# facebookresearch/dpr-scale

Measured on NVIDIA H100. Metric: query+ctx pairs/sec (BERT-base, seq128), higher is better.
Workload: dtype bf16

## Files before the change

dpr_scale_b200/csrc/common.cuh:

```cuda
#pragma once
#include <cuda.h>
#include <cuda_runtime.h>
#include <cuda_bf16.h>
#include <cuda_fp16.h>
#include <stdint.h>
#include "wgmma.cuh"

#ifndef DPRB_HANG_GUARD
#define DPRB_HANG_GUARD 1
#endif

namespace dprb {

typedef __nv_bfloat16 bf16;

void set_last_error(const char* fmt, ...);
#define DPRB_CHECK_CUDA(expr)                                                        \
  do {                                                                               \
    cudaError_t _e = (expr);                                                         \
    if (_e != cudaSuccess) {                                                         \
      dprb::set_last_error("%s:%d CUDA error %d (%s) in `%s`", __FILE__, __LINE__,   \
                           (int)_e, cudaGetErrorString(_e), #expr);                  \
      return 2;                                                                      \
    }                                                                                \
  } while (0)
#define DPRB_REQUIRE(cond, ...)                                                      \
  do {                                                                               \
    if (!(cond)) {                                                                   \
      dprb::set_last_error(__VA_ARGS__);                                             \
      return 1;                                                                      \
    }                                                                                \
  } while (0)

int num_sms();
#define DPRB_NUM_SMS(var)           \
  const int var = dprb::num_sms();  \
  if (var <= 0) return 2

void count_launch();
#define DPRB_LAUNCH_CHECK()                \
  do {                                     \
    dprb::count_launch();                  \
    DPRB_CHECK_CUDA(cudaGetLastError());   \
  } while (0)

__device__ __forceinline__ uint32_t smem_u32(const void* p) {
  return static_cast<uint32_t>(__cvta_generic_to_shared(p));
}
__device__ __forceinline__ uint8_t* align1024(uint8_t* p) {
  return reinterpret_cast<uint8_t*>((reinterpret_cast<uintptr_t>(p) + 1023) & ~uintptr_t(1023));
}
__device__ __forceinline__ void named_bar_sync(int id, int n) { asm volatile("bar.sync %0, %1;" ::"r"(id), "r"(n) : "memory"); }

__device__ __forceinline__ float warp_sum(float v) {
#pragma unroll
  for (int o = 16; o > 0; o >>= 1) v += __shfl_xor_sync(0xffffffffu, v, o);
  return v;
}
__device__ __forceinline__ float warp_max(float v) {
#pragma unroll
  for (int o = 16; o > 0; o >>= 1) v = fmaxf(v, __shfl_xor_sync(0xffffffffu, v, o));
  return v;
}

__device__ __forceinline__ uint32_t pack_bf16x2(float lo, float hi) {
  __nv_bfloat162 t = __floats2bfloat162_rn(lo, hi);
  return *reinterpret_cast<uint32_t*>(&t);
}
__device__ __forceinline__ float2 unpack_bf16x2(uint32_t u) {
  __nv_bfloat162 t = *reinterpret_cast<__nv_bfloat162*>(&u);
  return __bfloat1622float2(t);
}

__device__ __forceinline__ uint32_t pack_f16x2(float lo, float hi) {
  __half2 t = __floats2half2_rn(lo, hi);
  return *reinterpret_cast<uint32_t*>(&t);
}
__device__ __forceinline__ float2 unpack_f16x2(uint32_t u) {
  __half2 t = *reinterpret_cast<__half2*>(&u);
  return __half22float2(t);
}
__device__ __forceinline__ uint32_t pack_16x2(float lo, float hi, bool f16) { return f16 ? pack_f16x2(lo, hi) : pack_bf16x2(lo, hi); }
__device__ __forceinline__ float2 unpack_16x2(uint32_t u, bool f16) { return f16 ? unpack_f16x2(u) : unpack_bf16x2(u); }

__device__ __forceinline__ float2 ffma2(float2 a, float2 b, float2 c) {
  return make_float2(__fmaf_rn(a.x, b.x, c.x), __fmaf_rn(a.y, b.y, c.y));
}
__device__ __forceinline__ float2 fmul2(float2 a, float2 b) { return make_float2(__fmul_rn(a.x, b.x), __fmul_rn(a.y, b.y)); }
__device__ __forceinline__ float2 fadd2(float2 a, float2 b) { return make_float2(__fadd_rn(a.x, b.x), __fadd_rn(a.y, b.y)); }

__device__ __forceinline__ float ex2_approx(float x) {
  float y;
  asm("ex2.approx.ftz.f32 %0, %1;" : "=f"(y) : "f"(x));
  return y;
}
__device__ __forceinline__ float lg2_approx(float x) {
  float y;
  asm("lg2.approx.ftz.f32 %0, %1;" : "=f"(y) : "f"(x));
  return y;
}
__device__ __forceinline__ float rcp_approx(float x) {
  float y;
  asm("rcp.approx.ftz.f32 %0, %1;" : "=f"(y) : "f"(x));
  return y;
}
__device__ __forceinline__ void gelu_and_grad(float x, float& g, float& gd) {
  const float xc = fminf(fmaxf(x, -8.f), 8.f);
  const float x2 = xc * xc;
  float pz = fmaf(x2, 1.03455483e-3f, -1.06900513e-1f);
  pz = fmaf(pz, x2, -2.30098511f);
  const float e = ex2_approx(pz * xc);
  const float sg = rcp_approx(1.f + e);
  float zp = fmaf(x2, -3.58549371e-3f, 2.22293380e-1f);
  zp = fmaf(zp, x2, 1.59492135f);
  const float inside = (x == xc) ? zp : 0.f;
  g = x * sg;
  gd = sg * fmaf(xc * e * sg, inside, 1.f);
}
__device__ __forceinline__ void gelu_and_grad2(float2 x, float2& g, float2& gd) {
  float2 x2 = fmul2(x, x);
  x2.x = fminf(x2.x, 64.f);
  x2.y = fminf(x2.y, 64.f);
  const float2 one = make_float2(1.f, 1.f);
  float2 pz = ffma2(x2, make_float2(1.03455483e-3f, 1.03455483e-3f), make_float2(-1.06900513e-1f, -1.06900513e-1f));
  pz = ffma2(pz, x2, make_float2(-2.30098511f, -2.30098511f));
  const float2 ex = fmul2(pz, x);
  const float2 e = make_float2(ex2_approx(ex.x), ex2_approx(ex.y));
  const float2 den = fadd2(e, one);
  const float2 sg = make_float2(rcp_approx(den.x), rcp_approx(den.y));
  float2 zp = ffma2(x2, make_float2(-3.58549371e-3f, -3.58549371e-3f), make_float2(2.22293380e-1f, 2.22293380e-1f));
  zp = ffma2(zp, x2, make_float2(1.59492135f, 1.59492135f));
  g = fmul2(x, sg);
  const float2 t = ffma2(sg, make_float2(-1.f, -1.f), one);
  const float2 w = ffma2(fmul2(x, t), zp, one);
  gd = fmul2(sg, w);
}
struct Drop {
  uint32_t seed;
  uint32_t thresh16;
  float scale;
  uint32_t row_mul;
  __host__ __device__ bool on() const { return thresh16 != 0u; }
  __device__ __forceinline__ uint32_t group_mix(uint32_t r, uint32_t c8) const {
    uint32_t x = (r * row_mul) * 0x9E3779B1u + c8 * 0x85EBCA6Bu + seed;
    x ^= x >> 16; x *= 0x7FEB352Du; x ^= x >> 15;
    return x;
  }
  __device__ __forceinline__ static uint32_t pair_word(uint32_t x, uint32_t w) {
    const uint32_t k = w == 0u ? 0x846CA68Bu : (w == 1u ? 0xC2B2AE35u : (w == 2u ? 0x27D4EB2Fu : 0x165667B1u));
    uint32_t h = x * k;
    h ^= h >> 16;
    return h;
  }
  __device__ __forceinline__ uint32_t pair_hash(uint32_t r, uint32_t c_even) const {
    return pair_word(group_mix(r, c_even >> 3), (c_even >> 1) & 3u);
  }
  __device__ __forceinline__ void lanes(uint32_t h, float& m0, float& m1) const {
    m0 = (h & 0xFFFFu) >= thresh16 ? scale : 0.f;
    m1 = (h >> 16) >= thresh16 ? scale : 0.f;
  }
  __device__ __forceinline__ void mul2(uint32_t r, uint32_t c_even, float& m0, float& m1) const {
    lanes(pair_hash(r, c_even), m0, m1);
  }
  __device__ __forceinline__ void mul8(uint32_t r, uint32_t c0, float2 (&m)[4]) const {
    const uint32_t x = group_mix(r, c0 >> 3);
#pragma unroll
    for (int w = 0; w < 4; ++w) lanes(pair_word(x, (uint32_t)w), m[w].x, m[w].y);
  }
};
__device__ __forceinline__ float drop_one(const Drop& d, uint32_t r, uint32_t c) {
  float m0, m1;
  d.mul2(r, c & ~1u, m0, m1);
  return (c & 1u) ? m1 : m0;
}
inline Drop make_drop(float p, uint64_t seed, int layer, int site) {
  const uint64_t s64 = seed + (uint64_t)(layer * 8 + site + 1) * 0x9E3779B97F4A7C15ull;
  Drop d;
  d.seed = (uint32_t)(s64 ^ (s64 >> 32));
  d.thresh16 = (p > 0.f) ? (uint32_t)((double)p * 65536.0 + 0.5) : 0u;
  if (d.thresh16 > 65535u) d.thresh16 = 65535u;
  d.scale = d.thresh16 ? 1.f / (1.f - (float)d.thresh16 / 65536.f) : 1.f;
  d.row_mul = 1u;
  return d;
}
inline uint64_t drop_site_seed64(uint64_t seed, int layer, int site) { return make_drop(0.5f, seed, layer, site).seed; }
inline Drop drop_from_site(float p, uint64_t site_seed) {
  Drop d = make_drop(p, 0, 0, 0);
  d.seed = (uint32_t)site_seed;
  d.row_mul = (uint32_t)(site_seed >> 32) ? (uint32_t)(site_seed >> 32) : 1u;
  return d;
}
enum { DROP_SITE_EMBED = 0, DROP_SITE_ATTN = 1, DROP_SITE_ATTN_OUT = 2, DROP_SITE_FFN_OUT = 3,
       DROP_SITE_HEAD = 4, DROP_SITE_HEAD_IN = 5 };

__device__ __forceinline__ void mbar_init(uint64_t* bar, uint32_t count) {
  asm volatile("mbarrier.init.shared::cta.b64 [%0], %1;" ::"r"(smem_u32(bar)), "r"(count) : "memory");
}
__device__ __forceinline__ void fence_barrier_init() {
  asm volatile("fence.mbarrier_init.release.cluster;" ::: "memory");
}
__device__ __forceinline__ void fence_proxy_async_smem() {
  asm volatile("fence.proxy.async.shared::cta;" ::: "memory");
}
__device__ __forceinline__ void mbar_arrive_expect_tx(uint64_t* bar, uint32_t tx_bytes) {
  asm volatile("mbarrier.arrive.expect_tx.shared::cta.b64 _, [%0], %1;" ::"r"(smem_u32(bar)), "r"(tx_bytes)
// ... 86 lines not shown
```

dpr_scale_b200/csrc/gemm_wgmma.cu:

```cuda
#include <cstdlib>
#include <vector>
#include "common.cuh"
#include "dprb_internal.h"

namespace dprb {

namespace {

constexpr int BLOCK_M = 128;
constexpr int BLOCK_N = 256;
constexpr int BLOCK_K = 64;
constexpr int STAGES = 3;
constexpr int A_TILE_BYTES = BLOCK_M * BLOCK_K * 2;
constexpr int B_TILE_BYTES = BLOCK_N * BLOCK_K * 2;
constexpr int STAGE_BYTES = A_TILE_BYTES + B_TILE_BYTES;
constexpr int NUM_CONSUMERS = 2;
constexpr int NUM_THREADS = (NUM_CONSUMERS + 1) * 128;
constexpr int WG_ROWS = BLOCK_M / NUM_CONSUMERS;
constexpr int SUB_COLS = 64;
constexpr int SUB_BYTES = WG_ROWS * SUB_COLS * 2;
constexpr int STG_BYTES = WG_ROWS * BLOCK_N * 2;
constexpr int SMEM_BYTES = STAGES * STAGE_BYTES + NUM_CONSUMERS * STG_BYTES + 1024  + 128 ;
static_assert(SMEM_BYTES <= 227 * 1024, "ring + staging must fit one CTA per SM");
constexpr int PRODUCER_REGS = 40, CONSUMER_REGS = 232;
static_assert(128 * PRODUCER_REGS + NUM_CONSUMERS * 128 * CONSUMER_REGS <= 65536, "register file");

struct GemmParams {
  int M, N, K;
  int num_m_blocks, num_n_blocks;
  int k_blocks_total, k_blocks_per_split, splits;
  int units;
  int epilogue;
  void* D;
  long long ldd;
  const float* bias;
  int has_aux;
  int has_out2;
  float alpha;
  float* colsum;
  Drop drop;
  int aux_f16, out_f16;
  int save_pre;
};

struct Unit {
  int m0, n0, kb0, kb1;
};
__device__ __forceinline__ Unit unit_at(const GemmParams& p, int u) {
  const int tiles = p.num_m_blocks * p.num_n_blocks;
  const int tile = u % tiles, split = u / tiles;
  Unit w;
  w.m0 = (tile / p.num_n_blocks) * BLOCK_M;
  w.n0 = (tile % p.num_n_blocks) * BLOCK_N;
  w.kb0 = split * p.k_blocks_per_split;
  w.kb1 = min(w.kb0 + p.k_blocks_per_split, p.k_blocks_total);
  return w;
}

__device__ __forceinline__ void red_add_v2_f32(float* p, float a, float b) {
  asm volatile("red.global.add.v2.f32 [%0], {%1, %2};" ::"l"(p), "f"(a), "f"(b) : "memory");
}
__device__ __forceinline__ void wg_bar(int wg) { asm volatile("bar.sync %0, 128;" ::"r"(wg + 1) : "memory"); }

template <int A_MN, int B_MN, int F16>
__device__ __forceinline__ void mma_kblock(float (&acc)[128], uint32_t sa, uint32_t sb, int accumulate_first) {
  const uint64_t da = make_wgmma_desc_sw128(sa, A_MN ? BLOCK_K * 128 : 16, 1024);
  const uint64_t db = make_wgmma_desc_sw128(sb, B_MN ? BLOCK_K * 128 : 16, 1024);
  constexpr uint32_t A_KSTEP = (A_MN ? 16 * 128 : 32) >> 4;
  constexpr uint32_t B_KSTEP = (B_MN ? 16 * 128 : 32) >> 4;
#pragma unroll
  for (int k = 0; k < BLOCK_K / 16; ++k) {
    const int accum = (k > 0 || accumulate_first) ? 1 : 0;
    if (F16) wgmma_m64n256_ss_f16<A_MN, B_MN>(acc, da + k * A_KSTEP, db + k * B_KSTEP, accum);
    else wgmma_m64n256_ss_bf16<A_MN, B_MN>(acc, da + k * A_KSTEP, db + k * B_KSTEP, accum);
  }
}

__device__ __forceinline__ uint32_t pack_out(float a, float b, bool f16) { return f16 ? pack_f16x2(a, b) : pack_bf16x2(a, b); }

__device__ __forceinline__ uint32_t slab_base(const uint8_t* stg, int lr, int q) {
  return smem_u32(stg) + lr * 128 + ((lr & 7) << 4) + 4 * q;
}
__device__ __forceinline__ uint32_t slab_pair(uint32_t base, int c, int h) {
  return (base ^ ((c & 7) << 4)) + (c >> 3) * SUB_BYTES + h * 8 * 128;
}
__device__ __forceinline__ void sts32(uint32_t a, uint32_t v) { asm volatile("st.shared.b32 [%0], %1;" ::"r"(a), "r"(v)); }
__device__ __forceinline__ uint32_t lds32(uint32_t a) {
  uint32_t v;
  asm volatile("ld.shared.b32 %0, [%1];" : "=r"(v) : "r"(a));
  return v;
}
__device__ __forceinline__ int slab_boxes(int row0, int n0, int M, int N) {
  return row0 < M ? min(BLOCK_N / SUB_COLS, (N - n0 + SUB_COLS - 1) / SUB_COLS) : 0;
}
__device__ __forceinline__ void slab_tma_store(const CUtensorMap* m, const uint8_t* stg, int row0, int n0, int M, int N) {
  const int boxes = slab_boxes(row0, n0, M, N);
  for (int s = 0; s < boxes; ++s) tma_store_2d(m, smem_u32(stg + s * SUB_BYTES), n0 + s * SUB_COLS, row0);
  tma_store_commit();
}

template <bool ATOMIC>
__device__ __forceinline__ void epilogue_f32(const GemmParams& p, const float (&acc)[128], int row0, int n0, int lr, int q) {
#pragma unroll
  for (int h = 0; h < 2; ++h) {
    const int row = row0 + lr + 8 * h;
    if (row >= p.M) continue;
    float* drow = reinterpret_cast<float*>(p.D) + (long long)row * p.ldd;
#pragma unroll
    for (int c = 0; c < 32; ++c) {
      const int col = n0 + 8 * c + 2 * q;
      const float x = acc[4 * c + 2 * h] * p.alpha, y = acc[4 * c + 2 * h + 1] * p.alpha;
      if (ATOMIC) {
        if (col + 1 < p.N) red_add_v2_f32(drow + col, x, y);
        else if (col < p.N) atomicAdd(drow + col, x);
      } else {
        if (col < p.N) drow[col] = x + (p.bias != nullptr ? __ldg(p.bias + col) : 0.f);
        if (col + 1 < p.N) drow[col + 1] = y + (p.bias != nullptr ? __ldg(p.bias + col + 1) : 0.f);
      }
    }
  }
}

template <int EP, bool DROP, bool COLSUM>
__device__ __forceinline__ void epilogue16(const GemmParams& p, float (&acc)[128], uint32_t slab, int row0, int n0, int lr,
                                           int q, int lane) {
  const bool out_f16 = p.out_f16 != 0, aux_f16 = p.aux_f16 != 0;
#pragma unroll
  for (int c = 0; c < 32; ++c) {
    const int col = n0 + 8 * c + 2 * q;
    float2 b = make_float2(0.f, 0.f);
    if (p.bias != nullptr) {
      if (col + 1 < p.N) b = __ldg(reinterpret_cast<const float2*>(p.bias + col));
      else if (col < p.N) b.x = __ldg(p.bias + col);
    }
    float cs0 = 0.f, cs1 = 0.f;
#pragma unroll
    for (int h = 0; h < 2; ++h) {
      const int row = row0 + lr + 8 * h;
      const uint32_t sp = slab_pair(slab, c, h);
      float2 v = ffma2(make_float2(acc[4 * c + 2 * h], acc[4 * c + 2 * h + 1]), make_float2(p.alpha, p.alpha), b);
      if constexpr (EP == DPRB_EPI_BIAS_GELU) {
        float2 g, d;
        gelu_and_grad2(v, g, d);
        if (p.save_pre) d = v;
        sts32(sp, pack_bf16x2(g.x, g.y));
        acc[4 * c + 2 * h] = d.x;
        acc[4 * c + 2 * h + 1] = d.y;
        continue;
      }
      if constexpr (DROP) {
        float m0f, m1f;
        p.drop.mul2((uint32_t)row, (uint32_t)col, m0f, m1f);
        v.x *= m0f; v.y *= m1f;
      }
      if constexpr (EP == DPRB_EPI_BIAS_RESIDUAL) {
        const float2 a = unpack_16x2(lds32(sp), aux_f16);
        v.x += a.x; v.y += a.y;
      } else if constexpr (EP == DPRB_EPI_DGELU) {
        const float2 a = unpack_bf16x2(lds32(sp));
        v.x *= a.x; v.y *= a.y;
      } else if constexpr (EP == DPRB_EPI_DGELU_PRE) {
        float2 g, d;
        gelu_and_grad2(unpack_bf16x2(lds32(sp)), g, d);
        v.x *= d.x; v.y *= d.y;
      }
      const uint32_t o = pack_out(v.x, v.y, out_f16);
      sts32(sp, o);
      if (COLSUM && row < p.M && col < p.N) {
        const float2 f = unpack_bf16x2(o);
        cs0 += f.x;
        if (col + 1 < p.N) cs1 += f.y;
      }
    }
    if (COLSUM) {
#pragma unroll
      for (int o = 4; o < 32; o <<= 1) {
        cs0 += __shfl_xor_sync(0xFFFFFFFFu, cs0, o);
        cs1 += __shfl_xor_sync(0xFFFFFFFFu, cs1, o);
      }
      if (lane < 4) {
        if (col < p.N) atomicAdd(p.colsum + col, cs0);
        if (col + 1 < p.N) atomicAdd(p.colsum + col + 1, cs1);
      }
    }
  }
}

template <int A_MN, int B_MN, int F16>
__global__ void __launch_bounds__(NUM_THREADS, 1)
gemm_bf16_kernel(const __grid_constant__ CUtensorMap tmap_a, const __grid_constant__ CUtensorMap tmap_b,
                 const __grid_constant__ CUtensorMap tmap_d, const __grid_constant__ CUtensorMap tmap_aux,
                 const __grid_constant__ CUtensorMap tmap_out2, const GemmParams p) {
  extern __shared__ uint8_t smem_raw[];
  uint8_t* smem = align1024(smem_raw);
  uint8_t* staging = smem + STAGES * STAGE_BYTES;
  uint64_t* full_bar = reinterpret_cast<uint64_t*>(staging + NUM_CONSUMERS * STG_BYTES);
  uint64_t* empty_bar = full_bar + STAGES;
  uint64_t* aux_full = empty_bar + STAGES;
  uint64_t* slab_empty = aux_full + NUM_CONSUMERS;

  const int warp = threadIdx.x >> 5;
  const int lane = threadIdx.x & 31;
  const bool out16 = p.epilogue != DPRB_EPI_F32_ATOMIC_ADD && p.epilogue != DPRB_EPI_F32_STORE;

  if (threadIdx.x == 0) {
    tma_prefetch_desc(&tmap_a);
    tma_prefetch_desc(&tmap_b);
    if (out16) tma_prefetch_desc(&tmap_d);
    if (p.has_aux) tma_prefetch_desc(&tmap_aux);
    if (p.has_out2) tma_prefetch_desc(&tmap_out2);
    for (int i = 0; i < STAGES; ++i) {
      mbar_init(&full_bar[i], 1);
      mbar_init(&empty_bar[i], NUM_CONSUMERS * 4);
    }
    for (int i = 0; i < NUM_CONSUMERS; ++i) {
      mbar_init(&aux_full[i], 1);
      mbar_init(&slab_empty[i], 1);
    }
    fence_barrier_init();
  }
  __syncthreads();

  if (warp < 4) {
    asm volatile("setmaxnreg.dec.sync.aligned.u32 %0;" ::"n"(PRODUCER_REGS));
    if (warp == 0 && lane == 0) {
      int stage = 0;
      uint32_t phase = 0, uphase = 0;
      for (int u = blockIdx.x; u < p.units; u += gridDim.x, uphase ^= 1) {
        const Unit w = unit_at(p, u);
        const int aux_kb = min(w.kb0 + 2, w.kb1 - 1);
        for (int kb = w.kb0; kb < w.kb1; ++kb) {
          mbar_wait(&empty_bar[stage], phase ^ 1);
          mbar_arrive_expect_tx(&full_bar[stage], STAGE_BYTES);
          uint8_t* sa = smem + stage * STAGE_BYTES;
          uint8_t* sb = sa + A_TILE_BYTES;
          if (A_MN == 0) {
            tma_load_2d(sa, &tmap_a, &full_bar[stage], kb * BLOCK_K, w.m0);
          } else {
#pragma unroll
            for (int i = 0; i < BLOCK_M / 64; ++i) tma_load_2d(sa + i * (BLOCK_K * 128), &tmap_a, &full_bar[stage], w.m0 + i * 64, kb * BLOCK_K);
          }
          if (B_MN == 0) {
            tma_load_2d(sb, &tmap_b, &full_bar[stage], kb * BLOCK_K, w.n0);
          } else {
#pragma unroll
            for (int i = 0; i < BLOCK_N / 64; ++i) tma_load_2d(sb + i * (BLOCK_K * 128), &tmap_b, &full_bar[stage], w.n0 + i * 64, kb * BLOCK_K);
          }
          if (++stage == STAGES) { stage = 0; phase ^= 1; }
          if (p.has_aux && kb == aux_kb) {
            for (int g = 0; g < NUM_CONSUMERS; ++g) {
              const int row0 = w.m0 + g * WG_ROWS;
              const int boxes = slab_boxes(row0, w.n0, p.M, p.N);
              uint8_t* slab = staging + g * STG_BYTES;
              mbar_wait(&slab_empty[g], uphase);
              mbar_arrive_expect_tx(&aux_full[g], boxes * SUB_BYTES);
              for (int s = 0; s < boxes; ++s)
                tma_load_2d(slab + s * SUB_BYTES, &tmap_aux, &aux_full[g], w.n0 + s * SUB_COLS, row0);
            }
          }
        }
      }
    }
    return;
  }

  asm volatile("setmaxnreg.inc.sync.aligned.u32 %0;" ::"n"(CONSUMER_REGS));
  const int wg = (warp >> 2) - 1;
  const int t = threadIdx.x - 128 * (wg + 1);
  uint8_t* stg = staging + wg * STG_BYTES;
  const uint32_t a_off = (uint32_t)wg * (A_MN ? BLOCK_K * 128 : 64 * 128);
  const int q = lane & 3;
  const int lr = (warp & 3) * 16 + (lane >> 2);
  const uint32_t slab = slab_base(stg, lr, q);
  const int ep = p.epilogue;

  float acc[128];
  int stage = 0;
  uint32_t phase = 0, uphase = 0;
  for (int u = blockIdx.x; u < p.units; u += gridDim.x, uphase ^= 1) {
    const Unit w = unit_at(p, u);
    {
      int prev = -1;
      const int release_kb = min(w.kb0 + 1, w.kb1 - 1);
      for (int kb = w.kb0; kb < w.kb1; ++kb) {
        mbar_wait(&full_bar[stage], phase);
        const uint32_t sa = smem_u32(smem + stage * STAGE_BYTES) + a_off;
        const uint32_t sb = smem_u32(smem + stage * STAGE_BYTES + A_TILE_BYTES);
        wgmma_fence();
        mma_kblock<A_MN, B_MN, F16>(acc, sa, sb, kb > w.kb0);
        wgmma_commit();
        wgmma_wait<1>();
        if (prev >= 0) {
          __syncwarp();
          if (lane == 0) mbar_arrive(&empty_bar[prev]);
        }
        if (p.has_aux && kb == release_kb && t == 0) {
          tma_store_wait_read();
          mbar_arrive(&slab_empty[wg]);
        }
        prev = stage;
        if (++stage == STAGES) { stage = 0; phase ^= 1; }
      }
      wgmma_wait<0>();
      __syncwarp();
      if (lane == 0) mbar_arrive(&empty_bar[prev]);
    }

    const int row0 = w.m0 + wg * WG_ROWS;
    switch (ep) {
      case DPRB_EPI_F32_ATOMIC_ADD: epilogue_f32<true>(p, acc, row0, w.n0, lr, q); continue;
      case DPRB_EPI_F32_STORE: epilogue_f32<false>(p, acc, row0, w.n0, lr, q); continue;
      default: break;
    }
    if (p.has_aux) mbar_wait(&aux_full[wg], uphase);
    else if (t == 0) tma_store_wait_read();
    wg_bar(wg);
    const bool cs = p.colsum != nullptr, drop = p.drop.on();
    switch (ep) {
      case DPRB_EPI_BIAS:
        if (cs) epilogue16<DPRB_EPI_BIAS, false, true>(p, acc, slab, row0, w.n0, lr, q, lane);
        else epilogue16<DPRB_EPI_BIAS, false, false>(p, acc, slab, row0, w.n0, lr, q, lane);
        break;
      case DPRB_EPI_BIAS_GELU: epilogue16<DPRB_EPI_BIAS_GELU, false, false>(p, acc, slab, row0, w.n0, lr, q, lane); break;
      case DPRB_EPI_BIAS_RESIDUAL:
        if (drop) {
          if (cs) epilogue16<DPRB_EPI_BIAS_RESIDUAL, true, true>(p, acc, slab, row0, w.n0, lr, q, lane);
          else epilogue16<DPRB_EPI_BIAS_RESIDUAL, true, false>(p, acc, slab, row0, w.n0, lr, q, lane);
        } else {
          if (cs) epilogue16<DPRB_EPI_BIAS_RESIDUAL, false, true>(p, acc, slab, row0, w.n0, lr, q, lane);
          else epilogue16<DPRB_EPI_BIAS_RESIDUAL, false, false>(p, acc, slab, row0, w.n0, lr, q, lane);
        }
        break;
      case DPRB_EPI_DGELU:
        if (cs) epilogue16<DPRB_EPI_DGELU, false, true>(p, acc, slab, row0, w.n0, lr, q, lane);
        else epilogue16<DPRB_EPI_DGELU, false, false>(p, acc, slab, row0, w.n0, lr, q, lane);
        break;
      default:
        if (cs) epilogue16<DPRB_EPI_DGELU_PRE, false, true>(p, acc, slab, row0, w.n0, lr, q, lane);
        else epilogue16<DPRB_EPI_DGELU_PRE, false, false>(p, acc, slab, row0, w.n0, lr, q, lane);
        break;
    }
    fence_proxy_async_smem();
    wg_bar(wg);
    if (t == 0) slab_tma_store(&tmap_d, stg, row0, w.n0, p.M, p.N);
    if (p.has_out2) {
      if (t == 0) tma_store_wait_read();
      wg_bar(wg);
#pragma unroll
      for (int c = 0; c < 32; ++c)
#pragma unroll
        for (int h = 0; h < 2; ++h)
          sts32(slab_pair(slab, c, h), pack_bf16x2(acc[4 * c + 2 * h], acc[4 * c + 2 * h + 1]));
      fence_proxy_async_smem();
      wg_bar(wg);
      if (t == 0) slab_tma_store(&tmap_out2, stg, row0, w.n0, p.M, p.N);
    }
  }
  if (t == 0) tma_store_wait_all();
}

int make_tmap(CUtensorMap* out, const void* base, long long rows, long long cols, long long ld, int box_rows) {
  DPRB_REQUIRE((reinterpret_cast<uintptr_t>(base) & 15) == 0, "gemm operand base %p not 16-byte aligned", base);
  DPRB_REQUIRE((ld * 2) % 16 == 0, "gemm operand leading dimension %lld not a multiple of 8 elements", ld);
  const cuuint64_t dims[2] = {(cuuint64_t)cols, (cuuint64_t)rows};
  const cuuint64_t strides[1] = {(cuuint64_t)ld * 2};
  const cuuint32_t box[2] = {64u, (cuuint32_t)box_rows};
  return encode_tmap(out, "gemm", CU_TENSOR_MAP_DATA_TYPE_BFLOAT16, 2, base, dims, strides, box,
                     CU_TENSOR_MAP_L2_PROMOTION_L2_256B);
}

struct GemmProfile {
  bool enabled = false;
  std::vector<cudaEvent_t> ev;
  std::vector<double> flops;
  size_t used = 0;
};
GemmProfile g_prof;

int choose_splits(int tiles, int k_blocks, int sms) {
  int best = 1;
  double best_cost = 1e30;
  for (int s = 1; s <= 32; ++s) {
    if (k_blocks / s < 4 && s > 1) break;
    const int rounds = (tiles * s + sms - 1) / sms;
    const double cost = (double)rounds * ((k_blocks + s - 1) / s + 4);
    if (cost < best_cost - 1e-9) { best_cost = cost; best = s; }
  }
  return best;
}

}

int gemm_bf16(const void* A, const void* B, void* D, int M, int N, int K, long long lda, long long ldb,
              long long ldd, int a_mn_major, int b_mn_major, int epilogue, const float* bias, const void* aux,
              long long ld_aux, void* out2, float alpha, int splits, float* colsum, float dropout_p,
              unsigned long long drop_site_seed, cudaStream_t stream) {
  DPRB_REQUIRE(M > 0 && N > 0 && K > 0, "gemm: empty problem M=%d N=%d K=%d", M, N, K);
  const int dt_flags = epilogue & ~0xFF;
  epilogue &= 0xFF;
  const int a_f16 = (dt_flags & DPRB_GEMM_A_F16) != 0, b_f16 = (dt_flags & DPRB_GEMM_B_F16) != 0;
  const int aux_f16 = (dt_flags & DPRB_GEMM_AUX_F16) != 0, out_f16 = (dt_flags & DPRB_GEMM_OUT_F16) != 0;
  DPRB_REQUIRE(epilogue >= 0 && epilogue < DPRB_EPI_COUNT, "gemm: bad epilogue %d", epilogue);
  DPRB_REQUIRE(!(aux_f16 || out_f16) || epilogue == DPRB_EPI_BIAS || epilogue == DPRB_EPI_BIAS_RESIDUAL,
               "gemm: fp16 aux / output is implemented for the BIAS and BIAS_RESIDUAL epilogues only");
  DPRB_REQUIRE(a_f16 == b_f16, "gemm: wgmma takes no fp16 x bf16 operand pair: give "
               "DPRB_GEMM_A_F16 and DPRB_GEMM_B_F16 together or not at all");
  DPRB_REQUIRE(!out_f16 || colsum == nullptr, "gemm: colsum reads a bf16 slab (not available with fp16 output)");
  const bool f32_out = (epilogue == DPRB_EPI_F32_ATOMIC_ADD || epilogue == DPRB_EPI_F32_STORE);
  DPRB_REQUIRE(f32_out || (ldd % 8 == 0 && (reinterpret_cast<uintptr_t>(D) & 15) == 0),
               "gemm: bf16 output must be 16-byte aligned with ldd %% 8 == 0 (ldd=%lld)", ldd);
  DPRB_REQUIRE(!f32_out || (ldd % 4 == 0 && (reinterpret_cast<uintptr_t>(D) & 15) == 0),
               "gemm: fp32 output must be 16-byte aligned with ldd %% 4 == 0 (ldd=%lld)", ldd);
  const bool has_aux = epilogue == DPRB_EPI_BIAS_RESIDUAL || epilogue == DPRB_EPI_DGELU || epilogue == DPRB_EPI_DGELU_PRE;
  if (has_aux)
    DPRB_REQUIRE(aux != nullptr && ld_aux % 8 == 0 && (reinterpret_cast<uintptr_t>(aux) & 15) == 0,
                 "gemm: epilogue %d needs a 16-byte aligned aux with ld %% 8 == 0", epilogue);
  if (bias != nullptr) DPRB_REQUIRE((reinterpret_cast<uintptr_t>(bias) & 15) == 0, "gemm: bias not 16B aligned");

  DPRB_REQUIRE(colsum == nullptr || (!f32_out && epilogue != DPRB_EPI_BIAS_GELU),
               "gemm: colsum is supported for the BIAS / BIAS_RESIDUAL / DGELU epilogues only");

  const bool has_out2 = epilogue == DPRB_EPI_BIAS_GELU && out2 != nullptr;
  if (has_out2)
    DPRB_REQUIRE((reinterpret_cast<uintptr_t>(out2) & 15) == 0, "gemm: out2 not 16-byte aligned");

  CUtensorMap ta, tb, td{}, tx{}, to2{};
  int rc;
  if (!a_mn_major) rc = make_tmap(&ta, A, M, K, lda, BLOCK_M); else rc = make_tmap(&ta, A, K, M, lda, BLOCK_K);
  if (rc) return rc;
  if (!b_mn_major) rc = make_tmap(&tb, B, N, K, ldb, BLOCK_N); else rc = make_tmap(&tb, B, K, N, ldb, BLOCK_K);
  if (rc) return rc;
  if (!f32_out && (rc = make_tmap(&td, D, M, N, ldd, WG_ROWS))) return rc;
  if (has_aux && (rc = make_tmap(&tx, aux, M, N, ld_aux, WG_ROWS))) return rc;
  if (has_out2 && (rc = make_tmap(&to2, out2, M, N, ldd, WG_ROWS))) return rc;

  GemmParams p;
  p.M = M; p.N = N; p.K = K;
  p.num_m_blocks = (M + BLOCK_M - 1) / BLOCK_M;
  p.num_n_blocks = (N + BLOCK_N - 1) / BLOCK_N;
  p.k_blocks_total = (K + BLOCK_K - 1) / BLOCK_K;
  DPRB_NUM_SMS(sms);
  const int tiles = p.num_m_blocks * p.num_n_blocks;
  if (epilogue != DPRB_EPI_F32_ATOMIC_ADD) splits = 1;
  else if (splits <= 0) splits = choose_splits(tiles, p.k_blocks_total, sms);
  if (splits > p.k_blocks_total) splits = p.k_blocks_total;
  p.k_blocks_per_split = (p.k_blocks_total + splits - 1) / splits;
  p.splits = (p.k_blocks_total + p.k_blocks_per_split - 1) / p.k_blocks_per_split;
  p.epilogue = epilogue;
  p.D = D; p.ldd = ldd; p.bias = bias; p.has_aux = has_aux; p.has_out2 = has_out2; p.alpha = alpha;
  p.colsum = colsum;
  p.aux_f16 = aux_f16; p.out_f16 = out_f16;
  p.save_pre = (dt_flags & DPRB_GEMM_SAVE_PRE) != 0;
  p.drop = drop_from_site(epilogue == DPRB_EPI_BIAS_RESIDUAL ? dropout_p : 0.f, drop_site_seed);

  p.units = tiles * p.splits;
  const int grid = p.units < sms ? p.units : sms;
  static bool attr_set = false;
  if (!attr_set) {
#define DPRB_SET_ATTR(...) DPRB_CHECK_CUDA(cudaFuncSetAttribute(__VA_ARGS__, cudaFuncAttributeMaxDynamicSharedMemorySize, SMEM_BYTES));
    DPRB_SET_ATTR(gemm_bf16_kernel<0, 0, 0>) DPRB_SET_ATTR(gemm_bf16_kernel<0, 1, 0>)
    DPRB_SET_ATTR(gemm_bf16_kernel<1, 0, 0>) DPRB_SET_ATTR(gemm_bf16_kernel<1, 1, 0>)
    DPRB_SET_ATTR(gemm_bf16_kernel<0, 0, 1>) DPRB_SET_ATTR(gemm_bf16_kernel<0, 1, 1>)
    DPRB_SET_ATTR(gemm_bf16_kernel<1, 0, 1>) DPRB_SET_ATTR(gemm_bf16_kernel<1, 1, 1>)
#undef DPRB_SET_ATTR
    attr_set = true;
  }
  auto launch = [&](auto kern) -> int {
    const bool prof = g_prof.enabled && g_prof.used + 2 <= g_prof.ev.size();
    if (prof) DPRB_CHECK_CUDA(cudaEventRecord(g_prof.ev[g_prof.used], stream));
    kern<<<grid, NUM_THREADS, SMEM_BYTES, stream>>>(ta, tb, td, tx, to2, p);
    DPRB_LAUNCH_CHECK();
    if (prof) {
      DPRB_CHECK_CUDA(cudaEventRecord(g_prof.ev[g_prof.used + 1], stream));
      g_prof.flops.push_back(2.0 * (double)M * (double)N * (double)K);
      g_prof.used += 2;
    }
    return 0;
  };
  const int key = (a_mn_major ? 4 : 0) | (b_mn_major ? 2 : 0) | (a_f16 ? 1 : 0);
  switch (key) {
    case 0: return launch(gemm_bf16_kernel<0, 0, 0>);
    case 1: return launch(gemm_bf16_kernel<0, 0, 1>);
    case 2: return launch(gemm_bf16_kernel<0, 1, 0>);
    case 3: return launch(gemm_bf16_kernel<0, 1, 1>);
    case 4: return launch(gemm_bf16_kernel<1, 0, 0>);
    case 5: return launch(gemm_bf16_kernel<1, 0, 1>);
    case 6: return launch(gemm_bf16_kernel<1, 1, 0>);
    default: return launch(gemm_bf16_kernel<1, 1, 1>);
  }
}

int gemm_profile_enable(int enable, int max_launches) {
  if (enable) {
    const size_t want = (size_t)max_launches * 2;
    while (g_prof.ev.size() < want) {
      cudaEvent_t e;
      DPRB_CHECK_CUDA(cudaEventCreate(&e));
      g_prof.ev.push_back(e);
    }
    g_prof.used = 0;
    g_prof.flops.clear();
  }
  g_prof.enabled = enable != 0;
  return 0;
}

int gemm_profile_read(double* total_ms, double* total_flops, long long* launches) {
  double ms = 0.0, fl = 0.0;
  for (size_t i = 0; i + 1 < g_prof.used; i += 2) {
    DPRB_CHECK_CUDA(cudaEventSynchronize(g_prof.ev[i + 1]));
    float t = 0.f;
    DPRB_CHECK_CUDA(cudaEventElapsedTime(&t, g_prof.ev[i], g_prof.ev[i + 1]));
    ms += t;
    fl += g_prof.flops[i / 2];
  }
  if (total_ms) *total_ms = ms;
  if (total_flops) *total_flops = fl;
  if (launches) *launches = (long long)(g_prof.used / 2);
  return 0;
}

}
```

Measured before the change: 761.6.

## Add ping-pong WGMMA GEMM kernel with 128x128 tiles for small-K bf16 outputs

Adds a ping-pong GEMM kernel in which the two consumer warpgroups each own a whole 128x128 tile and alternate between mainloop and epilogue using ordered named barriers. One warpgroup's epilogue can then overlap the other's tensor-core work. A deeper 5-stage ring feeds it. It is selected for 16-bit-output GEMMs with K up to 768, which covers most BERT-base projections. Smaller N tiles raise tile counts and improve SM fill, at the cost of lower per-tile operand reuse and more complex barrier ordering.

```diff
diff --git a/dpr_scale_b200/csrc/common.cuh b/dpr_scale_b200/csrc/common.cuh
--- a/dpr_scale_b200/csrc/common.cuh
+++ b/dpr_scale_b200/csrc/common.cuh
@@ -51,6 +51,7 @@
   return reinterpret_cast<uint8_t*>((reinterpret_cast<uintptr_t>(p) + 1023) & ~uintptr_t(1023));
 }
 __device__ __forceinline__ void named_bar_sync(int id, int n) { asm volatile("bar.sync %0, %1;" ::"r"(id), "r"(n) : "memory"); }
+__device__ __forceinline__ void named_bar_arrive(int id, int n) { asm volatile("bar.arrive %0, %1;" ::"r"(id), "r"(n) : "memory"); }
 
 __device__ __forceinline__ float warp_sum(float v) {
 #pragma unroll
diff --git a/dpr_scale_b200/csrc/gemm_wgmma.cu b/dpr_scale_b200/csrc/gemm_wgmma.cu
--- a/dpr_scale_b200/csrc/gemm_wgmma.cu
+++ b/dpr_scale_b200/csrc/gemm_wgmma.cu
@@ -25,6 +25,15 @@
 constexpr int PRODUCER_REGS = 40, CONSUMER_REGS = 232;
 static_assert(128 * PRODUCER_REGS + NUM_CONSUMERS * 128 * CONSUMER_REGS <= 65536, "register file");
 
+constexpr int PP_BLOCK_N = 128;
+constexpr int PP_STAGES = 5;
+constexpr int PP_STAGE_BYTES = A_TILE_BYTES + PP_BLOCK_N * BLOCK_K * 2;
+constexpr int PP_STG_BYTES = BLOCK_M * PP_BLOCK_N * 2;
+constexpr int PP_SMEM_BYTES = PP_STAGES * PP_STAGE_BYTES + NUM_CONSUMERS * PP_STG_BYTES + 1024 + 128;
+static_assert(PP_SMEM_BYTES <= 227 * 1024, "ring + staging must fit one CTA per SM");
+constexpr int PP_MAX_K = 768;
+constexpr int ORDER_BAR = 3;
+
 struct GemmParams {
   int M, N, K;
   int num_m_blocks, num_n_blocks;
@@ -46,12 +55,13 @@
 struct Unit {
   int m0, n0, kb0, kb1;
 };
+template <int BN = BLOCK_N>
 __device__ __forceinline__ Unit unit_at(const GemmParams& p, int u) {
   const int tiles = p.num_m_blocks * p.num_n_blocks;
   const int tile = u % tiles, split = u / tiles;
   Unit w;
   w.m0 = (tile / p.num_n_blocks) * BLOCK_M;
-  w.n0 = (tile % p.num_n_blocks) * BLOCK_N;
+  w.n0 = (tile % p.num_n_blocks) * BN;
   w.kb0 = split * p.k_blocks_per_split;
   w.kb1 = min(w.kb0 + p.k_blocks_per_split, p.k_blocks_total);
   return w;
@@ -81,8 +91,9 @@
 __device__ __forceinline__ uint32_t slab_base(const uint8_t* stg, int lr, int q) {
   return smem_u32(stg) + lr * 128 + ((lr & 7) << 4) + 4 * q;
 }
-__device__ __forceinline__ uint32_t slab_pair(uint32_t base, int c, int h) {
-  return (base ^ ((c & 7) << 4)) + (c >> 3) * SUB_BYTES + h * 8 * 128;
+template <int MH>
+__device__ __forceinline__ uint32_t slab_pair(uint32_t base, int mh, int c, int h) {
+  return (base ^ ((c & 7) << 4)) + (c >> 3) * (MH * SUB_BYTES) + (64 * mh + 8 * h) * 128;
 }
 __device__ __forceinline__ void sts32(uint32_t a, uint32_t v) { asm volatile("st.shared.b32 [%0], %1;" ::"r"(a), "r"(v)); }
 __device__ __forceinline__ uint32_t lds32(uint32_t a) {
@@ -90,12 +101,15 @@
   asm volatile("ld.shared.b32 %0, [%1];" : "=r"(v) : "r"(a));
   return v;
 }
+template <int MH>
 __device__ __forceinline__ int slab_boxes(int row0, int n0, int M, int N) {
-  return row0 < M ? min(BLOCK_N / SUB_COLS, (N - n0 + SUB_COLS - 1) / SUB_COLS) : 0;
-}
+  constexpr int cols = MH == 1 ? BLOCK_N : PP_BLOCK_N;
+  return row0 < M ? min(cols / SUB_COLS, (N - n0 + SUB_COLS - 1) / SUB_COLS) : 0;
+}
+template <int MH>
 __device__ __forceinline__ void slab_tma_store(const CUtensorMap* m, const uint8_t* stg, int row0, int n0, int M, int N) {
-  const int boxes = slab_boxes(row0, n0, M, N);
-  for (int s = 0; s < boxes; ++s) tma_store_2d(m, smem_u32(stg + s * SUB_BYTES), n0 + s * SUB_COLS, row0);
+  const int boxes = slab_boxes<MH>(row0, n0, M, N);
+  for (int s = 0; s < boxes; ++s) tma_store_2d(m, smem_u32(stg + s * MH * SUB_BYTES), n0 + s * SUB_COLS, row0);
   tma_store_commit();
 }
 
@@ -121,12 +135,12 @@
   }
 }
 
-template <int EP, bool DROP, bool COLSUM>
-__device__ __forceinline__ void epilogue16(const GemmParams& p, float (&acc)[128], uint32_t slab, int row0, int n0, int lr,
-                                           int q, int lane) {
+template <int EP, bool DROP, bool COLSUM, int MH>
+__device__ __forceinline__ void epilogue16(const GemmParams& p, float (&acc)[MH][128 / MH], uint32_t slab, int row0, int n0,
+                                           int lr, int q, int lane) {
   const bool out_f16 = p.out_f16 != 0, aux_f16 = p.aux_f16 != 0;
 #pragma unroll
-  for (int c = 0; c < 32; ++c) {
+  for (int c = 0; c < 32 / MH; ++c) {
     const int col = n0 + 8 * c + 2 * q;
     float2 b = make_float2(0.f, 0.f);
     if (p.bias != nullptr) {
@@ -135,41 +149,45 @@
     }
     float cs0 = 0.f, cs1 = 0.f;
 #pragma unroll
-    for (int h = 0; h < 2; ++h) {
-      const int row = row0 + lr + 8 * h;
-      const uint32_t sp = slab_pair(slab, c, h);
-      float2 v = ffma2(make_float2(acc[4 * c + 2 * h], acc[4 * c + 2 * h + 1]), make_float2(p.alpha, p.alpha), b);
-      if constexpr (EP == DPRB_EPI_BIAS_GELU) {
-        float2 g, d;
-        gelu_and_grad2(v, g, d);
-        if (p.save_pre) d = v;
-        sts32(sp, pack_bf16x2(g.x, g.y));
-        acc[4 * c + 2 * h] = d.x;
-        acc[4 * c + 2 * h + 1] = d.y;
-        continue;
-      }
-      if constexpr (DROP) {
-        float m0f, m1f;
-        p.drop.mul2((uint32_t)row, (uint32_t)col, m0f, m1f);
-        v.x *= m0f; v.y *= m1f;
-      }
-      if constexpr (EP == DPRB_EPI_BIAS_RESIDUAL) {
-        const float2 a = unpack_16x2(lds32(sp), aux_f16);
-        v.x += a.x; v.y += a.y;
-      } else if constexpr (EP == DPRB_EPI_DGELU) {
-        const float2 a = unpack_bf16x2(lds32(sp));
-        v.x *= a.x; v.y *= a.y;
-      } else if constexpr (EP == DPRB_EPI_DGELU_PRE) {
-        float2 g, d;
-        gelu_and_grad2(unpack_bf16x2(lds32(sp)), g, d);
-        v.x *= d.x; v.y *= d.y;
-      }
-      const uint32_t o = pack_out(v.x, v.y, out_f16);
-      sts32(sp, o);
-      if (COLSUM && row < p.M && col < p.N) {
-        const float2 f = unpack_bf16x2(o);
-        cs0 += f.x;
-        if (col + 1 < p.N) cs1 += f.y;
+    for (int mh = 0; mh < MH; ++mh) {
+#pragma unroll
+      for (int h = 0; h < 2; ++h) {
+        const int row = row0 + 64 * mh + lr + 8 * h;
+        const uint32_t sp = slab_pair<MH>(slab, mh, c, h);
+        float* const d2 = &acc[mh][4 * c + 2 * h];
+        float2 v = ffma2(make_float2(d2[0], d2[1]), make_float2(p.alpha, p.alpha), b);
+        if constexpr (EP == DPRB_EPI_BIAS_GELU) {
+          float2 g, d;
+          gelu_and_grad2(v, g, d);
+          if (p.save_pre) d = v;
+          sts32(sp, pack_bf16x2(g.x, g.y));
+          d2[0] = d.x;
+          d2[1] = d.y;
+          continue;
+        }
+        if constexpr (DROP) {
+          float m0f, m1f;
+          p.drop.mul2((uint32_t)row, (uint32_t)col, m0f, m1f);
+          v.x *= m0f; v.y *= m1f;
+        }
+        if constexpr (EP == DPRB_EPI_BIAS_RESIDUAL) {
+          const float2 a = unpack_16x2(lds32(sp), aux_f16);
+          v.x += a.x; v.y += a.y;
+        } else if constexpr (EP == DPRB_EPI_DGELU) {
+          const float2 a = unpack_bf16x2(lds32(sp));
+          v.x *= a.x; v.y *= a.y;
+        } else if constexpr (EP == DPRB_EPI_DGELU_PRE) {
+          float2 g, d;
+          gelu_and_grad2(unpack_bf16x2(lds32(sp)), g, d);
+          v.x *= d.x; v.y *= d.y;
+        }
+        const uint32_t o = pack_out(v.x, v.y, out_f16);
+        sts32(sp, o);
+        if (COLSUM && row < p.M && col < p.N) {
+          const float2 f = unpack_bf16x2(o);
+          cs0 += f.x;
+          if (col + 1 < p.N) cs1 += f.y;
+        }
       }
     }
     if (COLSUM) {
@@ -183,6 +201,54 @@
         if (col + 1 < p.N) atomicAdd(p.colsum + col + 1, cs1);
       }
     }
+  }
+}
+
+template <int MH>
+__device__ __forceinline__ void store_tile16(const GemmParams& p, float (&acc)[MH][128 / MH], const CUtensorMap* tmap_d,
+                                             const CUtensorMap* tmap_out2, const uint8_t* stg, uint32_t slab, int row0,
+                                             int n0, int lr, int q, int lane, int t, int wg) {
+  const bool cs = p.colsum != nullptr, drop = p.drop.on();
+  switch (p.epilogue) {
+    case DPRB_EPI_BIAS:
+      if (cs) epilogue16<DPRB_EPI_BIAS, false, true>(p, acc, slab, row0, n0, lr, q, lane);
+      else epilogue16<DPRB_EPI_BIAS, false, false>(p, acc, slab, row0, n0, lr, q, lane);
+      break;
+    case DPRB_EPI_BIAS_GELU: epilogue16<DPRB_EPI_BIAS_GELU, false, false>(p, acc, slab, row0, n0, lr, q, lane); break;
+    case DPRB_EPI_BIAS_RESIDUAL:
+      if (drop) {
+        if (cs) epilogue16<DPRB_EPI_BIAS_RESIDUAL, true, true>(p, acc, slab, row0, n0, lr, q, lane);
+        else epilogue16<DPRB_EPI_BIAS_RESIDUAL, true, false>(p, acc, slab, row0, n0, lr, q, lane);
+      } else {
+        if (cs) epilogue16<DPRB_EPI_BIAS_RESIDUAL, false, true>(p, acc, slab, row0, n0, lr, q, lane);
+        else epilogue16<DPRB_EPI_BIAS_RESIDUAL, false, false>(p, acc, slab, row0, n0, lr, q, lane);
+      }
+      break;
+    case DPRB_EPI_DGELU:
+      if (cs) epilogue16<DPRB_EPI_DGELU, false, true>(p, acc, slab, row0, n0, lr, q, lane);
+      else epilogue16<DPRB_EPI_DGELU, false, false>(p, acc, slab, row0, n0, lr, q, lane);
+      break;
+    default:
+      if (cs) epilogue16<DPRB_EPI_DGELU_PRE, false, true>(p, acc, slab, row0, n0, lr, q, lane);
+      else epilogue16<DPRB_EPI_DGELU_PRE, false, false>(p, acc, slab, row0, n0, lr, q, lane);
+      break;
+  }
+  fence_proxy_async_smem();
+  wg_bar(wg);
+  if (t == 0) slab_tma_store<MH>(tmap_d, stg, row0, n0, p.M, p.N);
+  if (p.has_out2) {
+    if (t == 0) tma_store_wait_read();
+    wg_bar(wg);
+#pragma unroll
+    for (int c = 0; c < 32 / MH; ++c)
+#pragma unroll
+      for (int mh = 0; mh < MH; ++mh)
+#pragma unroll
+        for (int h = 0; h < 2; ++h)
+          sts32(slab_pair<MH>(slab, mh, c, h), pack_bf16x2(acc[mh][4 * c + 2 * h], acc[mh][4 * c + 2 * h + 1]));
+    fence_proxy_async_smem();
+    wg_bar(wg);
+    if (t == 0) slab_tma_store<MH>(tmap_out2, stg, row0, n0, p.M, p.N);
   }
 }
 
@@ -250,7 +316,7 @@
           if (p.has_aux && kb == aux_kb) {
             for (int g = 0; g < NUM_CONSUMERS; ++g) {
               const int row0 = w.m0 + g * WG_ROWS;
-              const int boxes = slab_boxes(row0, w.n0, p.M, p.N);
+              const int boxes = slab_boxes<1>(row0, w.n0, p.M, p.N);
               uint8_t* slab = staging + g * STG_BYTES;
               mbar_wait(&slab_empty[g], uphase);
               mbar_arrive_expect_tx(&aux_full[g], boxes * SUB_BYTES);
@@ -274,7 +340,7 @@
   const uint32_t slab = slab_base(stg, lr, q);
   const int ep = p.epilogue;
 
-  float acc[128];
+  float acc[1][128];
   int stage = 0;
   uint32_t phase = 0, uphase = 0;
   for (int u = blockIdx.x; u < p.units; u += gridDim.x, uphase ^= 1) {
@@ -287,7 +353,7 @@
         const uint32_t sa = smem_u32(smem + stage * STAGE_BYTES) + a_off;
         const uint32_t sb = smem_u32(smem + stage * STAGE_BYTES + A_TILE_BYTES);
         wgmma_fence();
-        mma_kblock<A_MN, B_MN, F16>(acc, sa, sb, kb > w.kb0);
+        mma_kblock<A_MN, B_MN, F16>(acc[0], sa, sb, kb > w.kb0);
         wgmma_commit();
         wgmma_wait<1>();
         if (prev >= 0) {
@@ -308,53 +374,158 @@
 
     const int row0 = w.m0 + wg * WG_ROWS;
     switch (ep) {
-      case DPRB_EPI_F32_ATOMIC_ADD: epilogue_f32<true>(p, acc, row0, w.n0, lr, q); continue;
-      case DPRB_EPI_F32_STORE: epilogue_f32<false>(p, acc, row0, w.n0, lr, q); continue;
+      case DPRB_EPI_F32_ATOMIC_ADD: epilogue_f32<true>(p, acc[0], row0, w.n0, lr, q); continue;
+      case DPRB_EPI_F32_STORE: epilogue_f32<false>(p, acc[0], row0, w.n0, lr, q); continue;
       default: break;
     }
     if (p.has_aux) mbar_wait(&aux_full[wg], uphase);
     else if (t == 0) tma_store_wait_read();
     wg_bar(wg);
-    const bool cs = p.colsum != nullptr, drop = p.drop.on();
-    switch (ep) {
-      case DPRB_EPI_BIAS:
-        if (cs) epilogue16<DPRB_EPI_BIAS, false, true>(p, acc, slab, row0, w.n0, lr, q, lane);
-        else epilogue16<DPRB_EPI_BIAS, false, false>(p, acc, slab, row0, w.n0, lr, q, lane);
-        break;
-      case DPRB_EPI_BIAS_GELU: epilogue16<DPRB_EPI_BIAS_GELU, false, false>(p, acc, slab, row0, w.n0, lr, q, lane); break;
-      case DPRB_EPI_BIAS_RESIDUAL:
-        if (drop) {
-          if (cs) epilogue16<DPRB_EPI_BIAS_RESIDUAL, true, true>(p, acc, slab, row0, w.n0, lr, q, lane);
-          else epilogue16<DPRB_EPI_BIAS_RESIDUAL, true, false>(p, acc, slab, row0, w.n0, lr, q, lane);
-        } else {
-          if (cs) epilogue16<DPRB_EPI_BIAS_RESIDUAL, false, true>(p, acc, slab, row0, w.n0, lr, q, lane);
-          else epilogue16<DPRB_EPI_BIAS_RESIDUAL, false, false>(p, acc, slab, row0, w.n0, lr, q, lane);
-        }
-        break;
-      case DPRB_EPI_DGELU:
-        if (cs) epilogue16<DPRB_EPI_DGELU, false, true>(p, acc, slab, row0, w.n0, lr, q, lane);
-        else epilogue16<DPRB_EPI_DGELU, false, false>(p, acc, slab, row0, w.n0, lr, q, lane);
-        break;
-      default:
-        if (cs) epilogue16<DPRB_EPI_DGELU_PRE, false, true>(p, acc, slab, row0, w.n0, lr, q, lane);
-        else epilogue16<DPRB_EPI_DGELU_PRE, false, false>(p, acc, slab, row0, w.n0, lr, q, lane);
-        break;
-    }
-    fence_proxy_async_smem();
+    store_tile16<1>(p, acc, &tmap_d, &tmap_out2, stg, slab, row0, w.n0, lr, q, lane, t, wg);
+  }
+  if (t == 0) tma_store_wait_all();
+}
+
+template <int A_MN, int B_MN, int F16>
+__device__ __forceinline__ void mma_kblock_128x128(float (&acc)[2][64], uint32_t sa, uint32_t sb, int accumulate_first) {
+  const uint64_t da = make_wgmma_desc_sw128(sa, A_MN ? BLOCK_K * 128 : 16, 1024);
+  const uint64_t db = make_wgmma_desc_sw128(sb, B_MN ? BLOCK_K * 128 : 16, 1024);
+  constexpr uint32_t A_KSTEP = (A_MN ? 16 * 128 : 32) >> 4;
+  constexpr uint32_t B_KSTEP = (B_MN ? 16 * 128 : 32) >> 4;
+  constexpr uint32_t A_HALF = (64 * 128) >> 4;
+  static_assert(BLOCK_K * 128 == 64 * 128, "rows [64, 128) of A sit 8 KB in for both layouts");
+#pragma unroll
+  for (int k = 0; k < BLOCK_K / 16; ++k) {
+    const int accum = (k > 0 || accumulate_first) ? 1 : 0;
+#pragma unroll
+    for (int mh = 0; mh < 2; ++mh) {
+      if (F16) wgmma_m64n128_ss_f16<A_MN, B_MN>(acc[mh], da + mh * A_HALF + k * A_KSTEP, db + k * B_KSTEP, accum);
+      else wgmma_m64n128_ss_bf16<A_MN, B_MN>(acc[mh], da + mh * A_HALF + k * A_KSTEP, db + k * B_KSTEP, accum);
+    }
+  }
+}
+
+template <int A_MN, int B_MN, int F16>
+__global__ void __launch_bounds__(NUM_THREADS, 1)
+gemm16_pingpong_kernel(const __grid_constant__ CUtensorMap tmap_a, const __grid_constant__ CUtensorMap tmap_b,
+                       const __grid_constant__ CUtensorMap tmap_d, const __grid_constant__ CUtensorMap tmap_aux,
+                       const __grid_constant__ CUtensorMap tmap_out2, const GemmParams p) {
+  extern __shared__ uint8_t smem_raw[];
+  uint8_t* smem = align1024(smem_raw);
+  uint8_t* staging = smem + PP_STAGES * PP_STAGE_BYTES;
+  uint64_t* full_bar = reinterpret_cast<uint64_t*>(staging + NUM_CONSUMERS * PP_STG_BYTES);
+  uint64_t* empty_bar = full_bar + PP_STAGES;
+  uint64_t* aux_full = empty_bar + PP_STAGES;
+  uint64_t* slab_empty = aux_full + NUM_CONSUMERS;
+
+  const int warp = threadIdx.x >> 5;
+  const int lane = threadIdx.x & 31;
+
+  if (threadIdx.x == 0) {
+    tma_prefetch_desc(&tmap_a);
+    tma_prefetch_desc(&tmap_b);
+    tma_prefetch_desc(&tmap_d);
+    if (p.has_aux) tma_prefetch_desc(&tmap_aux);
+    if (p.has_out2) tma_prefetch_desc(&tmap_out2);
+    for (int i = 0; i < PP_STAGES; ++i) {
+      mbar_init(&full_bar[i], 1);
+      mbar_init(&empty_bar[i], 4);
+    }
+    for (int i = 0; i < NUM_CONSUMERS; ++i) {
+      mbar_init(&aux_full[i], 1);
+      mbar_init(&slab_empty[i], 1);
+    }
+    fence_barrier_init();
+  }
+  __syncthreads();
+
+  if (warp < 4) {
+    asm volatile("setmaxnreg.dec.sync.aligned.u32 %0;" ::"n"(PRODUCER_REGS));
+    if (warp == 0 && lane == 0) {
+      int stage = 0;
+      uint32_t phase = 0;
+      for (int u = blockIdx.x, i = 0; u < p.units; u += gridDim.x, ++i) {
+        const Unit w = unit_at<PP_BLOCK_N>(p, u);
+        const int g = i & 1;
+        const int aux_kb = min(w.kb0 + 2, w.kb1 - 1);
+        for (int kb = w.kb0; kb < w.kb1; ++kb) {
+          mbar_wait(&empty_bar[stage], phase ^ 1);
+          mbar_arrive_expect_tx(&full_bar[stage], PP_STAGE_BYTES);
+          uint8_t* sa = smem + stage * PP_STAGE_BYTES;
+          uint8_t* sb = sa + A_TILE_BYTES;
+          if (A_MN == 0) {
+            tma_load_2d(sa, &tmap_a, &full_bar[stage], kb * BLOCK_K, w.m0);
+          } else {
+#pragma unroll
+            for (int j = 0; j < BLOCK_M / 64; ++j) tma_load_2d(sa + j * (BLOCK_K * 128), &tmap_a, &full_bar[stage], w.m0 + j * 64, kb * BLOCK_K);
+          }
+          if (B_MN == 0) {
+            tma_load_2d(sb, &tmap_b, &full_bar[stage], kb * BLOCK_K, w.n0);
+          } else {
+#pragma unroll
+            for (int j = 0; j < PP_BLOCK_N / 64; ++j) tma_load_2d(sb + j * (BLOCK_K * 128), &tmap_b, &full_bar[stage], w.n0 + j * 64, kb * BLOCK_K);
+          }
+          if (++stage == PP_STAGES) { stage = 0; phase ^= 1; }
+          if (p.has_aux && kb == aux_kb) {
+            const int boxes = slab_boxes<2>(w.m0, w.n0, p.M, p.N);
+            uint8_t* slab = staging + g * PP_STG_BYTES;
+            mbar_wait(&slab_empty[g], (i >> 1) & 1);
+            mbar_arrive_expect_tx(&aux_full[g], boxes * 2 * SUB_BYTES);
+            for (int s = 0; s < boxes; ++s)
+              tma_load_2d(slab + s * 2 * SUB_BYTES, &tmap_aux, &aux_full[g], w.n0 + s * SUB_COLS, w.m0);
+          }
+        }
+      }
+    }
+    return;
+  }
+
+  asm volatile("setmaxnreg.inc.sync.aligned.u32 %0;" ::"n"(CONSUMER_REGS));
+  const int wg = (warp >> 2) - 1;
+  const int t = threadIdx.x - 128 * (wg + 1);
+  uint8_t* stg = staging + wg * PP_STG_BYTES;
+  const int q = lane & 3;
+  const int lr = (warp & 3) * 16 + (lane >> 2);
+  const uint32_t slab = slab_base(stg, lr, q);
+  const int unit_kbs = p.k_blocks_total;
+  uint32_t ring = (uint32_t)(wg * unit_kbs);
+
+  float acc[2][64];
+  uint32_t uphase = 0;
+  for (int u = blockIdx.x + wg * gridDim.x; u < p.units; u += NUM_CONSUMERS * gridDim.x, uphase ^= 1, ring += unit_kbs) {
+    const Unit w = unit_at<PP_BLOCK_N>(p, u);
+    if (u != (int)blockIdx.x) named_bar_sync(ORDER_BAR + wg, NUM_CONSUMERS * 128);
+    {
+      int prev = -1;
+      const int release_kb = min(w.kb0 + 1, w.kb1 - 1);
+      for (int kb = w.kb0; kb < w.kb1; ++kb, ++ring) {
+        const int stage = ring % PP_STAGES;
+        mbar_wait(&full_bar[stage], (ring / PP_STAGES) & 1);
+        const uint32_t sa = smem_u32(smem + stage * PP_STAGE_BYTES);
+        wgmma_fence();
+        mma_kblock_128x128<A_MN, B_MN, F16>(acc, sa, sa + A_TILE_BYTES, kb > w.kb0);
+        wgmma_commit();
+        wgmma_wait<1>();
+        if (prev >= 0) {
+          __syncwarp();
+          if (lane == 0) mbar_arrive(&empty_bar[prev]);
+        }
+        if (p.has_aux && kb == release_kb && t == 0) {
+          tma_store_wait_read();
+          mbar_arrive(&slab_empty[wg]);
+        }
+        prev = stage;
+      }
+      if (u + (int)gridDim.x < p.units) named_bar_arrive(ORDER_BAR + (wg ^ 1), NUM_CONSUMERS * 128);
+      wgmma_wait<0>();
+      __syncwarp();
+      if (lane == 0) mbar_arrive(&empty_bar[prev]);
+    }
+
+    if (p.has_aux) mbar_wait(&aux_full[wg], uphase);
+    else if (t == 0) tma_store_wait_read();
     wg_bar(wg);
-    if (t == 0) slab_tma_store(&tmap_d, stg, row0, w.n0, p.M, p.N);
-    if (p.has_out2) {
-      if (t == 0) tma_store_wait_read();
-      wg_bar(wg);
-#pragma unroll
-      for (int c = 0; c < 32; ++c)
-#pragma unroll
-        for (int h = 0; h < 2; ++h)
-          sts32(slab_pair(slab, c, h), pack_bf16x2(acc[4 * c + 2 * h], acc[4 * c + 2 * h + 1]));
-      fence_proxy_async_smem();
-      wg_bar(wg);
-      if (t == 0) slab_tma_store(&tmap_out2, stg, row0, w.n0, p.M, p.N);
-    }
+    store_tile16<2>(p, acc, &tmap_d, &tmap_out2, stg, slab, w.m0, w.n0, lr, q, lane, t, wg);
   }
   if (t == 0) tma_store_wait_all();
 }
@@ -424,20 +595,23 @@
   if (has_out2)
     DPRB_REQUIRE((reinterpret_cast<uintptr_t>(out2) & 15) == 0, "gemm: out2 not 16-byte aligned");
 
+  const bool pingpong = !f32_out && K <= PP_MAX_K;
+  const int block_n = pingpong ? PP_BLOCK_N : BLOCK_N;
+  const int slab_rows = pingpong ? BLOCK_M : WG_ROWS;
   CUtensorMap ta, tb, td{}, tx{}, to2{};
   int rc;
   if (!a_mn_major) rc = make_tmap(&ta, A, M, K, lda, BLOCK_M); else rc = make_tmap(&ta, A, K, M, lda, BLOCK_K);
   if (rc) return rc;
-  if (!b_mn_major) rc = make_tmap(&tb, B, N, K, ldb, BLOCK_N); else rc = make_tmap(&tb, B, K, N, ldb, BLOCK_K);
+  if (!b_mn_major) rc = make_tmap(&tb, B, N, K, ldb, block_n); else rc = make_tmap(&tb, B, K, N, ldb, BLOCK_K);
   if (rc) return rc;
-  if (!f32_out && (rc = make_tmap(&td, D, M, N, ldd, WG_ROWS))) return rc;
-  if (has_aux && (rc = make_tmap(&tx, aux, M, N, ld_aux, WG_ROWS))) return rc;
-  if (has_out2 && (rc = make_tmap(&to2, out2, M, N, ldd, WG_ROWS))) return rc;
+  if (!f32_out && (rc = make_tmap(&td, D, M, N, ldd, slab_rows))) return rc;
+  if (has_aux && (rc = make_tmap(&tx, aux, M, N, ld_aux, slab_rows))) return rc;
+  if (has_out2 && (rc = make_tmap(&to2, out2, M, N, ldd, slab_rows))) return rc;
 
   GemmParams p;
   p.M = M; p.N = N; p.K = K;
   p.num_m_blocks = (M + BLOCK_M - 1) / BLOCK_M;
-  p.num_n_blocks = (N + BLOCK_N - 1) / BLOCK_N;
+  p.num_n_blocks = (N + block_n - 1) / block_n;
   p.k_blocks_total = (K + BLOCK_K - 1) / BLOCK_K;
   DPRB_NUM_SMS(sms);
   const int tiles = p.num_m_blocks * p.num_n_blocks;
@@ -463,12 +637,18 @@
     DPRB_SET_ATTR(gemm_bf16_kernel<0, 0, 1>) DPRB_SET_ATTR(gemm_bf16_kernel<0, 1, 1>)
     DPRB_SET_ATTR(gemm_bf16_kernel<1, 0, 1>) DPRB_SET_ATTR(gemm_bf16_kernel<1, 1, 1>)
 #undef DPRB_SET_ATTR
+#define DPRB_SET_ATTR(...) DPRB_CHECK_CUDA(cudaFuncSetAttribute(__VA_ARGS__, cudaFuncAttributeMaxDynamicSharedMemorySize, PP_SMEM_BYTES));
+    DPRB_SET_ATTR(gemm16_pingpong_kernel<0, 0, 0>) DPRB_SET_ATTR(gemm16_pingpong_kernel<0, 1, 0>)
+    DPRB_SET_ATTR(gemm16_pingpong_kernel<1, 0, 0>) DPRB_SET_ATTR(gemm16_pingpong_kernel<1, 1, 0>)
+    DPRB_SET_ATTR(gemm16_pingpong_kernel<0, 0, 1>) DPRB_SET_ATTR(gemm16_pingpong_kernel<0, 1, 1>)
+    DPRB_SET_ATTR(gemm16_pingpong_kernel<1, 0, 1>) DPRB_SET_ATTR(gemm16_pingpong_kernel<1, 1, 1>)
+#undef DPRB_SET_ATTR
     attr_set = true;
   }
-  auto launch = [&](auto kern) -> int {
+  auto launch = [&](auto kern, int smem_bytes) -> int {
     const bool prof = g_prof.enabled && g_prof.used + 2 <= g_prof.ev.size();
     if (prof) DPRB_CHECK_CUDA(cudaEventRecord(g_prof.ev[g_prof.used], stream));
-    kern<<<grid, NUM_THREADS, SMEM_BYTES, stream>>>(ta, tb, td, tx, to2, p);
+    kern<<<grid, NUM_THREADS, smem_bytes, stream>>>(ta, tb, td, tx, to2, p);
     DPRB_LAUNCH_CHECK();
     if (prof) {
       DPRB_CHECK_CUDA(cudaEventRecord(g_prof.ev[g_prof.used + 1], stream));
@@ -478,15 +658,27 @@
     return 0;
   };
   const int key = (a_mn_major ? 4 : 0) | (b_mn_major ? 2 : 0) | (a_f16 ? 1 : 0);
+  if (pingpong) {
+    switch (key) {
+      case 0: return launch(gemm16_pingpong_kernel<0, 0, 0>, PP_SMEM_BYTES);
+      case 1: return launch(gemm16_pingpong_kernel<0, 0, 1>, PP_SMEM_BYTES);
+      case 2: return launch(gemm16_pingpong_kernel<0, 1, 0>, PP_SMEM_BYTES);
+      case 3: return launch(gemm16_pingpong_kernel<0, 1, 1>, PP_SMEM_BYTES);
+      case 4: return launch(gemm16_pingpong_kernel<1, 0, 0>, PP_SMEM_BYTES);
+      case 5: return launch(gemm16_pingpong_kernel<1, 0, 1>, PP_SMEM_BYTES);
+      case 6: return launch(gemm16_pingpong_kernel<1, 1, 0>, PP_SMEM_BYTES);
+      default: return launch(gemm16_pingpong_kernel<1, 1, 1>, PP_SMEM_BYTES);
+    }
+  }
   switch (key) {
-    case 0: return launch(gemm_bf16_kernel<0, 0, 0>);
-    case 1: return launch(gemm_bf16_kernel<0, 0, 1>);
-    case 2: return launch(gemm_bf16_kernel<0, 1, 0>);
-    case 3: return launch(gemm_bf16_kernel<0, 1, 1>);
-    case 4: return launch(gemm_bf16_kernel<1, 0, 0>);
-    case 5: return launch(gemm_bf16_kernel<1, 0, 1>);
-    case 6: return launch(gemm_bf16_kernel<1, 1, 0>);
-    default: return launch(gemm_bf16_kernel<1, 1, 1>);
+    case 0: return launch(gemm_bf16_kernel<0, 0, 0>, SMEM_BYTES);
+    case 1: return launch(gemm_bf16_kernel<0, 0, 1>, SMEM_BYTES);
+    case 2: return launch(gemm_bf16_kernel<0, 1, 0>, SMEM_BYTES);
+    case 3: return launch(gemm_bf16_kernel<0, 1, 1>, SMEM_BYTES);
+    case 4: return launch(gemm_bf16_kernel<1, 0, 0>, SMEM_BYTES);
+    case 5: return launch(gemm_bf16_kernel<1, 0, 1>, SMEM_BYTES);
+    case 6: return launch(gemm_bf16_kernel<1, 1, 0>, SMEM_BYTES);
+    default: return launch(gemm_bf16_kernel<1, 1, 1>, SMEM_BYTES);
   }
 }
 
```

Measured after the change: 772.1, median of 6. +1.4%, better.
